# Dzh-16/FLASH-Viterbi

Hardware: AMD Instinct MI355X
Metric: trellis_cells_per_sec (higher is better)
Workload: dtype f32 scores (+f64 add per cell, rounded to f32 as the reference does)

## Files before the change

flash_viterbi_amd/build.py:

```python
import os
import shutil
import subprocess

PKG = os.path.dirname(os.path.abspath(__file__))
ROOT = os.path.dirname(PKG)
INCLUDE = os.path.join(ROOT, "include")
CSRC = os.path.join(PKG, "csrc")

HOST_LIB = os.path.join(PKG, "libfvhost.so")
HIP_LIB = os.path.join(PKG, "libflashvit.so")

HIP_SOURCES = ["fv_context.hip", "fv_full.hip", "fv_beam.hip", "fv_comm.hip", "fv_schedule.cpp"]
HIP_DEPS = ["fv_internal.h", "fv_layout.h", "fv_device_common.h", "fv_kernels.hip.inc", "fv_beam_kernels.hip.inc", "fv_schedule.h"]
OBJ_DIR = os.path.join(PKG, "_obj")
HIP_TIMING_LIB = os.path.join(PKG, "libflashvit_timing.so")


def _newer(target, sources):
    if not os.path.isfile(target):
        return False
    t = os.path.getmtime(target)
    return all(os.path.getmtime(s) <= t for s in sources if os.path.isfile(s))


def _run(cmd, cwd=None):
    res = subprocess.run(cmd, cwd=cwd, capture_output=True, text=True)
    if res.returncode != 0:
        raise RuntimeError("build failed: " + " ".join(cmd) + "\n" + res.stdout + res.stderr)
# ... 73 lines not shown
```

flash_viterbi_amd/csrc/fv_context.hip:

```cpp
#include "fv_internal.h"

namespace {

template <typename F>
void parallel_rows(int rows, F &&fn)
{
    unsigned hw = std::thread::hardware_concurrency();
    int nt = (int)std::min<unsigned>(hw ? hw : 4, 16);
    if (rows < 256) nt = 1;
    if (nt <= 1) { fn(0, rows); return; }
    std::vector<std::thread> th;
    int per = (rows + nt - 1) / nt;
    for (int t = 0; t < nt; ++t) {
        int a = t * per, b = std::min(rows, a + per);
        if (a >= b) break;
        th.emplace_back([=, &fn] { fn(a, b); });
    }
    for (auto &x : th) x.join();
}

}

namespace fvi {

size_t device_bytes(const fv_ctx *c)
{
    return c->LA32.bytes() + c->LA16.bytes() + c->LAQ16.bytes() + c->SPdata.bytes() + c->SPoff.bytes() + c->SPnwb.bytes() + c->LB32T.bytes() + c->LA64.bytes() + c->LB64T.bytes() + c->LPi64.bytes() +
           c->d_ob.bytes() + c->d_ans.bytes() + c->d_bp.bytes() + c->d_gather.bytes() + c->d_rows.bytes() + c->d_ckpt.bytes() +
           c->d_score.bytes() + c->d_counters.bytes() + c->d_hval.bytes() + c->d_scores.bytes() +
           c->d_hstate.bytes() + c->d_flags.bytes() + c->d_slot_val.bytes() + c->d_slot_state.bytes() +
           c->LA64R.bytes() + c->LAQ16R.bytes() + c->d_qaux.bytes() + c->d_tie_list.bytes() + c->d_tie_count.bytes() + c->d_cut.bytes() + c->d_dupwin.bytes() + c->d_cand.bytes() + c->d_cand_count.bytes() + c->d_passL.bytes() + c->d_needfull.bytes() + c->d_seqof.bytes() + c->d_doubt.bytes() + c->d_doubt_count.bytes() + c->d_pack.bytes() +
           c->CSk.bytes() + c->CSq.bytes() + c->CS64.bytes() + c->CSoff.bytes() + c->CSnwb.bytes() + c->CRptr.bytes() + c->CRcol.bytes() + c->CRlog.bytes();
}

inline size_t pack_head(int nscores) { return 2 * FV_NCOUNTERS + (size_t)std::max(4, round_up(nscores, 4)); }

size_t pack_ints(const fv_ctx *ctx, int T, int nscores) { return pack_head(nscores) + (size_t)T * std::max(1, ctx->nranks) + (size_t)T; }

int ensure_workspace(fv_ctx *ctx, int T, size_t rows_needed, int nscores)
{
    const size_t want_rows = rows_needed * 2 * (size_t)ctx->nrows;
    const size_t want_pack = pack_ints(ctx, T, nscores);
    if (nscores > 1) {
        unsigned long long grow = 0, released = 0;
// ... 231 lines not shown
        for (fv_ctx *m : g->members) m->group = nullptr;
        for (size_t r = g->members.size(); r-- > 1;) fv_destroy(g->members[r]);
        for (hipEvent_t e : g->ans_ready) if (e) (void)hipEventDestroy(e);
        delete g;
    }
    (void)hipSetDevice(ctx->device);
    if (ctx->stream) (void)hipStreamSynchronize(ctx->stream);
    if (ctx->comm) ncclCommDestroy(ctx->comm);
    ctx->LA32.release(); ctx->LA16.release(); ctx->LAQ16.release(); ctx->SPdata.release(); ctx->SPoff.release(); ctx->SPnwb.release(); ctx->LB32T.release(); ctx->LA64.release(); ctx->LB64T.release(); ctx->LPi64.release();
    ctx->d_ob.release(); ctx->d_ans.release(); ctx->d_bp.release(); ctx->d_gather.release(); ctx->d_rows.release(); ctx->d_ckpt.release();
    ctx->d_score.release(); ctx->d_counters.release(); ctx->d_hval.release(); ctx->d_scores.release();
    ctx->d_hstate.release(); ctx->d_flags.release(); ctx->d_slot_val.release(); ctx->d_slot_state.release();
    ctx->LA64R.release(); ctx->LAQ16R.release(); ctx->d_qaux.release(); ctx->d_tie_list.release(); ctx->d_tie_count.release(); ctx->d_cut.release(); ctx->d_dupwin.release(); ctx->d_cand.release(); ctx->d_cand_count.release(); ctx->d_passL.release(); ctx->d_needfull.release(); ctx->d_seqof.release(); ctx->d_doubt.release(); ctx->d_doubt_count.release(); ctx->d_pack.release();
    fvi::release_csr(ctx);
    if (ctx->h_pin) { (void)hipHostFree(ctx->h_pin); ctx->h_pin = nullptr; ctx->h_pin_n = 0; }
    for (hipEvent_t e : ctx->prof_events) (void)hipEventDestroy(e);
    if (ctx->ev_start) (void)hipEventDestroy(ctx->ev_start);
    if (ctx->ev_stop) (void)hipEventDestroy(ctx->ev_stop);
    if (ctx->ev_top) (void)hipEventDestroy(ctx->ev_top);
    if (ctx->ev_s0) (void)hipEventDestroy(ctx->ev_s0);
    if (ctx->ev_s1) (void)hipEventDestroy(ctx->ev_s1);
    if (ctx->ev_fork) (void)hipEventDestroy(ctx->ev_fork);
    for (int q = 0; q < fv_ctx::BEAM_AUX; ++q) {
        if (ctx->ev_join[q]) (void)hipEventDestroy(ctx->ev_join[q]);
        if (ctx->aux[q]) (void)hipStreamDestroy(ctx->aux[q]);
    }
    if (ctx->stream) (void)hipStreamDestroy(ctx->stream);
    delete ctx;
}

// ... 400 lines not shown
    if (ctx->group && ctx->group_rank == 0) {
        for (int r = fvi::group_size(ctx) - 1; r >= 1; --r) {
            const int rc = fv_set_option(fvi::group_member(ctx, r), key, value);
            if (rc) return rc;
        }
    }
    switch (key) {
    case FV_OPT_KERNEL:
        if (value < FV_KERNEL_AUTO || value > FV_KERNEL_U16_REFINE) return FV_ERR_ARG;
        ctx->opt_kernel = (int)value; return FV_OK;
    case FV_OPT_MAX_BATCH:
        if (value < 1 || value > fvk::MAX_BATCH) return FV_ERR_ARG;
        ctx->opt_max_batch = (int)value; return FV_OK;
    case FV_OPT_PROFILE:
        ctx->opt_profile = value ? 1 : 0; return FV_OK;
    case FV_OPT_SEL_MARGIN:
        if (value < 0 || value > 100000) return FV_ERR_ARG;
        ctx->opt_sel_margin = (float)value * 1e-3f; return FV_OK;
    case FV_OPT_DEBUG:
#ifndef FV_TIMING_BUILD
        if (value & FV_DEBUG_TIMING_ONLY) { ctx->detail = "FV_OPT_DEBUG: result-changing timing switches need the timing build"; return FV_ERR_ARG; }
#endif
        if (value < 0 || value >= (1ll << 32) || (value & ((1ll << 27) | (1ll << 30)))) return FV_ERR_ARG;
        ctx->opt_csr_mem = (int)((value >> 31) & 1);
        ctx->opt_debug = (int)(value & 0x3fffffff); return FV_OK;
    default: return FV_ERR_ARG;
    }
}

extern "C" long long fv_checkpoint_memory_bytes(int K, int T, int step)
// ... 50 lines not shown
```

flash_viterbi_amd/csrc/fv_full.hip:

```cpp
#include "fv_internal.h"
#include "fv_kernels.hip.inc"
#include "flashvit_testing.h"

namespace {

int pick_kernel(const fv_ctx *ctx)
{
    if (ctx->opt_kernel == FV_KERNEL_F64_STREAM) return FV_KERNEL_F64_STREAM;
    if (!ctx->logs_nonpositive) return FV_KERNEL_F64_STREAM;
    if (ctx->opt_kernel == FV_KERNEL_F16_REFINE || ctx->opt_kernel == FV_KERNEL_F32_REFINE ||
        ctx->opt_kernel == FV_KERNEL_Q16_REFINE || ctx->opt_kernel == FV_KERNEL_U16_REFINE)
        return ctx->opt_kernel;
    if (ctx->opt_kernel == FV_KERNEL_SPARSE_Q16) return ctx->SPdata.p ? FV_KERNEL_SPARSE_Q16 : FV_KERNEL_U16_REFINE;
    return (ctx->SPdata.p && ctx->density <= 0.35) ? FV_KERNEL_SPARSE_Q16 : FV_KERNEL_U16_REFINE;
}

constexpr int U_UP = 16, U_DB32 = 4, U_DB64 = 2, U_DB16 = 2;

constexpr int nb_slot(int NB) { return NB == 1 ? 0 : NB == 2 ? 1 : NB == 4 ? 2 : 3; }
template <typename TA> constexpr int tab_slot()
{
    return std::is_same<TA, double>::value ? 0 : std::is_same<TA, float>::value ? 1 : std::is_same<TA, fvk::half_t>::value ? 2 : 3;
}
template <typename TA, int NB, bool DB> constexpr unsigned long long step_variant()
// ... 255 lines not shown

struct ProfRange { size_t first, count; };

int prof_event(fv_ctx *ctx, size_t idx, hipEvent_t *out)
{
    while (ctx->prof_events.size() <= idx) {
        hipEvent_t e;
        FV_HIP(hipEventCreate(&e));
        ctx->prof_events.push_back(e);
    }
    *out = ctx->prof_events[idx];
    return 0;
}

enum { BATCH_NONE = 0, BATCH_SERIAL = 1, BATCH_FORK = 2 };
int run_generation_full(fv_ctx *ctx, std::vector<fv::Pass> &passes, int kernel, size_t &nprof, int batch = BATCH_NONE)
{
    const int K = ctx->K;
    const int np = (int)passes.size();
    if (np == 0) return 0;
    std::stable_sort(passes.begin(), passes.end(),
                     [](const fv::Pass &a, const fv::Pass &b) { return a.R - a.L > b.R - b.L; });
    for (int base = 0; base < np; base += fvk::PASS_CHUNK) {
        fvk::PassChunk ch;
        ch.n = std::min(fvk::PASS_CHUNK, np - base);
        for (int q = 0; q < ch.n; ++q) {
            const fv::Pass &p = passes[base + q];
            ch.p[q] = fvk::PassDesc{ p.L, p.R, p.from_pi ? 1 : 0, p.whole ? 1 : 0, (long long)(base + q) * 2 * ctx->nrows };
        }
        if (ctx->csr)
            hipLaunchKernelGGL(fvk::init_rows_csr, dim3((K + 255) / 256, ch.n), dim3(256), 0, ctx->stream, ch, ctx->CRptr.p,
                               ctx->CRcol.p, ctx->CRlog.p, ctx->LB64T.p, ctx->LPi64.p, ctx->d_ob.p, ctx->d_ans.p, ctx->d_rows.p, K);
        else
        hipLaunchKernelGGL(fvk::init_rows, dim3((K + 255) / 256, ch.n), dim3(256), 0, ctx->stream, ch,
                           ctx->LA64.p, ctx->nrows, ctx->LB64T.p, ctx->LPi64.p, ctx->d_ob.p, ctx->d_ans.p,
                           ctx->d_rows.p, K);
        FV_HIP(hipGetLastError());
    }
    const int maxlen = passes[0].R - passes[0].L;
    const bool slabbed = (kernel == FV_KERNEL_F64_STREAM || kernel == FV_KERNEL_Q16_REFINE) && !ctx->full_ok;
    int cap = std::max(1, std::min(ctx->opt_max_batch, slabbed ? 4 : max_batch_for(ctx->nrows, !ctx->full_ok)));
    if (kernel == FV_KERNEL_SPARSE_CSR) cap = ctx->opt_max_batch;
    const bool whole_gen = passes[0].whole;
    constexpr int FORK_STREAMS = 3, FORK_CAP = 4;
    const bool two = ((kernel == FV_KERNEL_U16_REFINE && ctx->u16_ok) || ((kernel == FV_KERNEL_SPARSE_Q16 || kernel == FV_KERNEL_SPARSE_CSR) && maxlen >= 64)) &&
                     !(ctx->opt_debug & 262144) && (!whole_gen || batch == BATCH_FORK) && np > FORK_CAP &&
                     !ctx->opt_profile && !(ctx->opt_debug & 64);
    const int nbatches = (np + FORK_CAP - 1) / FORK_CAP;
    const int nstreams = two ? std::min(FORK_STREAMS, nbatches) : 1;
    auto fork = [&]() -> int {
        FV_HIP(hipEventRecord(ctx->ev_fork, ctx->stream));
        for (int q = 1; q < nstreams; ++q) FV_HIP(hipStreamWaitEvent(ctx->aux[q - 1], ctx->ev_fork, 0));
        return 0;
// ... 5 lines not shown
            while ((qe = hipStreamQuery(ctx->stream)) == hipErrorNotReady) std::this_thread::yield();
            FV_HIP(qe);
        }
        ctx->fork_active = true;
        { int rc = fork(); if (rc) return rc; }
    }
    ctx->forked_batches = two;
    struct Unfork { fv_ctx *c; ~Unfork() { c->forked_batches = false; c->lstream = nullptr; } } unfork{ ctx };
    auto join = [&]() -> int {
        for (int q = 1; q < nstreams; ++q) {
            FV_HIP(hipEventRecord(ctx->ev_join[q - 1], ctx->aux[q - 1]));
            FV_HIP(hipStreamWaitEvent(ctx->stream, ctx->ev_join[q - 1], 0));
        }
        return 0;
    };
    const bool col_last = !(ctx->opt_debug & 8);
    const bool use_graph = (ctx->opt_debug & 64) && !ctx->opt_profile;
    if (use_graph) FV_HIP(hipStreamBeginCapture(ctx->stream, hipStreamCaptureModeThreadLocal));
    if (whole_gen && !use_graph) FV_HIP(hipEventRecord(ctx->ev_s0, ctx->stream));
    int active = np;
    for (int s = 1; s <= maxlen; ++s) {
        while (active > 0 && passes[active - 1].R - passes[active - 1].L < s) --active;
        int full = active;
        if (col_last) while (full > 0 && passes[full - 1].R - passes[full - 1].L == s && !passes[full - 1].whole) --full;
        auto row = [&](int q, int parity) { return ctx->d_rows.p + (size_t)q * 2 * ctx->nrows + (size_t)parity * ctx->nrows; };
        for (int base = 0; base < full; base += cap) {
            const int nb = std::min(cap, full - base);
            fvk::TaskSlot slots[fvk::MAX_BATCH];
            for (int q = 0; q < nb; ++q) {
                const fv::Pass &p = passes[base + q];
                slots[q].t1_in = row(base + q, (s - 1) & 1);
                slots[q].t1_out = row(base + q, s & 1);
                slots[q].tmp_row = ctx->LB32T.p + (size_t)ctx->h_ob[p.L + s] * K;
                slots[q].tmp64_row = ctx->LB64T.p + (size_t)ctx->h_ob[p.L + s] * K;
                slots[q].bp_out = ctx->d_bp.p + (size_t)(p.L + s) * K;
            }
// ... 41 lines not shown
            }
            int rc = flush();
            if (rc) return rc;
        }
    }
    if (use_graph) {
        hipGraph_t g = nullptr;
        FV_HIP(hipStreamEndCapture(ctx->stream, &g));
        hipGraphExec_t ge = nullptr;
        FV_HIP(hipGraphInstantiate(&ge, g, nullptr, nullptr, 0));
        if (whole_gen) FV_HIP(hipEventRecord(ctx->ev_s0, ctx->stream));
        FV_HIP(hipGraphLaunch(ge, ctx->stream));
        ctx->graphs.push_back(ge);
        (void)hipGraphDestroy(g);
    }
    if (whole_gen && !two) FV_HIP(hipEventRecord(ctx->ev_s1, ctx->stream));
    if (two) { int rc = join(); if (rc) return rc; }
    if (whole_gen && two) FV_HIP(hipEventRecord(ctx->ev_s1, ctx->stream));
    if (batch) {
        fvk::ArgmaxArgs a;
        a.rows = ctx->d_rows.p; a.ans = ctx->d_ans.p; a.score = ctx->d_score.p; a.K = K; a.nrows = ctx->nrows; a.n = 0;
        auto flush = [&]() -> int {
            if (a.n == 0) return 0;
            hipLaunchKernelGGL(fvk::final_argmax_batch, dim3(a.n), dim3(1024), 0, ctx->stream, a);
            FV_HIP(hipGetLastError());
            a.n = 0;
            return 0;
        };
        for (int q = 0; q < np; ++q) {
            if (!passes[q].whole) continue;
            const int len = passes[q].R - passes[q].L;
// ... 297 lines not shown
    for (int q = 0; q < np; ++q) {
        const fv::Pass &p = gen[(size_t)q];
        int c = 0;
        while (tp[c].L != p.L) ++c;
        const float *row = ctx->d_rows.p + (size_t)q * 2 * ctx->nrows + (size_t)((p.R - p.L) & 1) * ctx->nrows;
        FV_HIP(hipMemcpyAsync(rows_out + (size_t)c * K, row, (size_t)K * sizeof(float), hipMemcpyDeviceToHost, ctx->stream));
        FV_HIP(hipMemcpyAsync(bp_out + (size_t)(p.L + 1) * K, ctx->d_bp.p + (size_t)(p.L + 1) * K,
                              (size_t)(p.R - p.L) * K * sizeof(int), hipMemcpyDeviceToHost, ctx->stream));
    }
    FV_HIP(hipStreamSynchronize(ctx->stream));
    for (hipGraphExec_t ge : ctx->graphs) (void)hipGraphExecDestroy(ge);
    ctx->graphs.clear();
    if (variants_out) *variants_out = ctx->test_variants;
    return FV_OK;
}
}

extern "C" int fv_test_forward(fv_ctx *ctx, const int *ob, int T, const fv_test_pass *passes, int npasses,
                               float *rows_out, int *bp_out, unsigned long long *variants_out)
{
    if (!ctx) return FV_ERR_ARG;
    if (fvi::group_size(ctx) > 1) { ctx->detail = "fv_test_forward: one device per context"; return FV_ERR_ARG; }
    return fvi::drained(ctx, test_forward_impl(ctx, ob, T, passes, npasses, rows_out, bp_out, variants_out));
}

extern "C" int fv_decode_vanilla(fv_ctx *ctx, const int *ob, int T, int *path_out, float *score_out)
{
    if (!ctx) return FV_ERR_ARG;
    if (ctx->csr) { ctx->detail = "fv_decode_vanilla: not available on a model set by fv_set_model_sparse (its kernel reads the dense table)"; return FV_ERR_UNSUPPORTED; }
    const int keep_kernel = ctx->opt_kernel;
// ... 112 lines not shown
```

flash_viterbi_amd/csrc/fv_internal.h:

```cpp
#pragma once

#include <hip/hip_runtime.h>
#include <rccl/rccl.h>

#include <algorithm>
#include <chrono>
#include <condition_variable>
#include <functional>
#include <mutex>
#include <cmath>
#include <cstdio>
#include <cstdlib>
#include <cstring>
#include <string>
#include <thread>
#include <vector>

#include "flashvit.h"
#include "fv_layout.h"
#include "fv_schedule.h"

using clk = std::chrono::steady_clock;
inline double ms_since(clk::time_point t0) { return std::chrono::duration<double, std::milli>(clk::now() - t0).count(); }

// ... 42 lines not shown
    bool laq16_ready = false;
    DevBuf<double> LA64, LB64T, LPi64;
    bool csr = false;
    DevBuf<uint4> CSk;
    DevBuf<uint2> CSq;
    DevBuf<double> CS64;
    DevBuf<long long> CSoff;
    DevBuf<int> CSnwb;
    DevBuf<long long> CRptr;
    DevBuf<int> CRcol;
    DevBuf<double> CRlog;

    DevBuf<int> d_ob, d_ans, d_bp, d_gather;
    DevBuf<float> d_rows, d_score, d_ckpt;
    DevBuf<unsigned long long> d_counters;
    DevBuf<int> d_pack;
    int *h_pin = nullptr;
    size_t h_pin_n = 0;
    DevBuf<float> d_hval, d_scores, d_slot_val;
    DevBuf<int> d_hstate, d_slot_state, d_flags;
    DevBuf<double> LA64R;
    DevBuf<unsigned short> LAQ16R;
    bool rowq_ready = false, beam_q16_ready = false;
    DevBuf<unsigned long long> d_qaux;
    DevBuf<int2> d_tie_list;
    DevBuf<float> d_cut;
    DevBuf<fvb::HNode> d_cand;
    DevBuf<int> d_cand_count;
    float opt_sel_margin = 0.3f;
    DevBuf<int> d_dupwin;
    DevBuf<int> d_doubt, d_doubt_count;
    DevBuf<int> d_needfull;
    DevBuf<int> d_seqof;
    std::vector<int> h_seqof;
    DevBuf<int> d_passL;
    std::vector<int> h_passL;
    DevBuf<unsigned int> d_tie_count;

    int opt_kernel = FV_KERNEL_AUTO;
    int opt_max_batch = fvk::MAX_BATCH;
    int opt_profile = 0;
    int vanilla = 0;
    int opt_csr_mem = 0;
    int opt_debug = 0;
    std::vector<hipEvent_t> prof_events;
    std::vector<int> h_ob;
    std::vector<hipGraphExec_t> graphs;
    bool test_record = false;
    unsigned long long test_variants = 0;

    ncclComm_t comm = nullptr;
    int rank = 0, nranks = 1;
    struct fv_group *group = nullptr;
    int group_rank = 0;

    fv_stats stats{};
// ... 76 lines not shown
```

flash_viterbi_amd/decoder.py:

```python
import ctypes
import os

import numpy as np

from . import build as _build

MODE_REFERENCE = 0
MODE_SINGLE_PASS = 1
KERNEL_AUTO, KERNEL_F64_STREAM, KERNEL_F32_REFINE, KERNEL_F16_REFINE, KERNEL_Q16_REFINE, KERNEL_SPARSE_Q16 = 0, 1, 2, 3, 4, 5
KERNEL_U16_REFINE = 6
KERNEL_SPARSE_CSR = 7
OPT_KERNEL, OPT_MAX_BATCH, OPT_PROFILE, OPT_SEL_MARGIN, OPT_DEBUG = 1, 2, 3, 4, 100
DEBUG_TIMING_ONLY = (1 << 0) | (1 << 4) | (1 << 5) | (1 << 11) | (1 << 12)
DEBUG_BATCH_GEN0_SERIAL = 1 << 28
DEBUG_BEAM_BATCH_GEN0_OTHER = 1 << 29
DEBUG_CSR_ROWS_IN_MEMORY = 1 << 31
WARN_BEAM_MISS = 1
ERR_ARG, ERR_NOMEM, ERR_NO_PRED, ERR_DEVICE, ERR_STATE, ERR_UNSUPPORTED = -1, -2, -3, -4, -5, -6
UNIQUE_ID_BYTES = 128


class Stats(ctypes.Structure):
    _fields_ = [("set_model_ms", ctypes.c_double), ("decode_ms", ctypes.c_double), ("gpu_ms", ctypes.c_double),
                ("top_pass_ms", ctypes.c_double), ("top_steps_ms", ctypes.c_double),
                ("step_kernel_ms", ctypes.c_double),
                ("step_launches", ctypes.c_longlong), ("task_steps", ctypes.c_longlong),
                ("column_steps", ctypes.c_longlong),
# ... 11 lines not shown

    def as_dict(self):
        return {k: getattr(self, k) for k, _ in self._fields_}


class PassInfo(ctypes.Structure):
    _fields_ = [("L", ctypes.c_int), ("R", ctypes.c_int), ("generation", ctypes.c_int), ("owner", ctypes.c_int)]


EXPORTS = ["fv_create", "fv_destroy", "fv_set_model", "fv_set_option", "fv_decode_full", "fv_decode_beam",
           "fv_decode_vanilla", "fv_decode_checkpoint", "fv_checkpoint_memory_bytes",
           "fv_last_stats", "fv_strerror", "fv_last_error_detail", "fv_reference_memory_bytes",
           "fv_comm_unique_id", "fv_comm_init", "fv_plan_passes", "fv_merge_paths", "fv_set_partition",
           "fv_create_multi", "fv_device_count", "fv_decode_full_batch", "fv_plan_passes_batch", "fv_decode_beam_batch",
           "fv_set_model_sparse"]
TEST_EXPORTS = ["fv_test_forward", "fv_test_beam_step"]
TIE_TAG = 1 << 30


class ForwardPass(ctypes.Structure):
    _fields_ = [("L", ctypes.c_int), ("R", ctypes.c_int), ("init_state", ctypes.c_int)]


class BeamSet(ctypes.Structure):
    _fields_ = [("val", ctypes.c_void_p), ("state", ctypes.c_void_p), ("n", ctypes.c_int)]

_lib = None


def load_library():
    global _lib
# ... 23 lines not shown
    L.fv_checkpoint_memory_bytes.argtypes = [ci, ci, ci]
    L.fv_checkpoint_memory_bytes.restype = ctypes.c_longlong
    L.fv_last_stats.argtypes = [vp, ctypes.POINTER(Stats)]
    L.fv_strerror.argtypes = [ci]
    L.fv_strerror.restype = ctypes.c_char_p
    L.fv_last_error_detail.argtypes = [vp]
    L.fv_last_error_detail.restype = ctypes.c_char_p
    L.fv_reference_memory_bytes.argtypes = [ci, ci, ci, ci]
    L.fv_reference_memory_bytes.restype = cll
    L.fv_comm_unique_id.argtypes = [vp]
    L.fv_comm_init.argtypes = [vp, ci, ci, vp]
    L.fv_set_partition.argtypes = [vp, ci, ci]
    L.fv_plan_passes.argtypes = [ci, ci, ci, ci, ctypes.POINTER(PassInfo), ci]
    L.fv_merge_paths.argtypes = [ci, ci, ci, vp, vp]
    L.fv_test_forward.argtypes = [vp, vp, ci, ctypes.POINTER(ForwardPass), ci, vp, vp, ctypes.POINTER(ctypes.c_ulonglong)]
    cf = ctypes.c_float
    L.fv_test_beam_step.argtypes = [vp, ci, ctypes.POINTER(BeamSet), ci, vp, ci, cf, cf, ci, vp, vp, vp, ctypes.POINTER(ci),
                                    vp, vp, vp, vp, ctypes.POINTER(ctypes.c_ulonglong)]
    _lib = L
    return L


class FlashVitError(RuntimeError):
    def __init__(self, rc, detail=""):
        msg = load_library().fv_strerror(rc).decode()
        super().__init__(f"flashvit: {msg} ({rc})" + (f": {detail}" if detail else ""))
        self.rc = rc


def plan_passes(T, n_split, mode=MODE_REFERENCE, nranks=1):
# ... 150 lines not shown
    def decode_checkpoint(self, ob, step=0):
        ob = np.ascontiguousarray(ob, dtype=np.int32)
        path = np.empty(ob.size, dtype=np.int32)
        score = ctypes.c_float(0)
        rc = self._check(self._L.fv_decode_checkpoint(self._h, _p(ob), ob.size, step, _p(path), ctypes.byref(score)))
        return path, np.float32(score.value), rc

    def test_forward(self, ob, passes, bp_fill=-2):
        ob = np.ascontiguousarray(ob, dtype=np.int32)
        pa = (ForwardPass * len(passes))(*[ForwardPass(int(L), int(R), int(s)) for L, R, s in passes])
        rows = np.empty((len(passes), self.K), dtype=np.float32)
        bp = np.full((ob.size, self.K), bp_fill, dtype=np.int32)
        variants = ctypes.c_ulonglong(0)
        self._check(self._L.fv_test_forward(self._h, _p(ob), ob.size, pa, len(passes), _p(rows), _p(bp), ctypes.byref(variants)))
        return rows, bp, int(variants.value)

    def test_beam_step(self, beam, sets, syms, speculative=False, theta=0.0, next_bound=float("inf"), cand_cap=0):
        K = self.K
        vals = [np.ascontiguousarray(v, dtype=np.float32) for v, _ in sets]
        sts = [np.ascontiguousarray(s, dtype=np.int32) for _, s in sets]
        arr = (BeamSet * len(sets))(*[BeamSet(_p(v).value, _p(s).value, v.size) for v, s in zip(vals, sts)])
        syms = np.ascontiguousarray(syms, dtype=np.int32)
        n = len(sets)
        scores = np.empty((n, K), dtype=np.float32)
        bp = np.empty((n, K), dtype=np.int32)
        ties = np.empty((n * K, 2), dtype=np.int32)
        nties = ctypes.c_int(0)
        doubt = np.empty((n, 1024), dtype=np.int32)
        doubt_counts = np.empty(n, dtype=np.int32)
        cand = np.empty((n, max(cand_cap, 1), 2), dtype=np.int32)
# ... 38 lines not shown
```

include/flashvit.h:

```cpp
#ifndef FLASHVIT_H
#define FLASHVIT_H

#include <stddef.h>

#ifdef __cplusplus
extern "C" {
#endif

typedef struct fv_ctx fv_ctx;

enum {
    FV_OK = 0,
    FV_WARN_BEAM_MISS = 1,
    FV_ERR_ARG = -1,
    FV_ERR_NOMEM = -2,
    FV_ERR_NO_PRED = -3,
    FV_ERR_DEVICE = -4,
    FV_ERR_STATE = -5,
    FV_ERR_UNSUPPORTED = -6,
    FV_ERR_COMM = -7,
};

enum {
    FV_MODE_REFERENCE = 0,
    FV_MODE_SINGLE_PASS = 1,
};

enum {
    FV_OPT_KERNEL = 1,
    FV_OPT_MAX_BATCH = 2,
    FV_OPT_PROFILE = 3,
    FV_OPT_SEL_MARGIN = 4,
    FV_OPT_DEBUG = 100,
};
#define FV_DEBUG_TIMING_ONLY ((1 << 0) | (1 << 4) | (1 << 5) | (1 << 11) | (1 << 12))
enum {
    FV_KERNEL_AUTO = 0,
    FV_KERNEL_F64_STREAM = 1,
    FV_KERNEL_F32_REFINE = 2,
    FV_KERNEL_F16_REFINE = 3,
    FV_KERNEL_Q16_REFINE = 4,
    FV_KERNEL_U16_REFINE = 6,
    FV_KERNEL_SPARSE_Q16 = 5,
    FV_KERNEL_SPARSE_CSR = 7,
};

typedef struct {
// ... 88 lines not shown
```

include/flashvit_testing.h:

```cpp
#ifndef FLASHVIT_TESTING_H
#define FLASHVIT_TESTING_H

#include "flashvit.h"

#ifdef __cplusplus
extern "C" {
#endif

typedef struct { int L, R, init_state; } fv_test_pass;

int fv_test_forward(fv_ctx *ctx, const int *ob, int T, const fv_test_pass *passes, int npasses,
                    float *rows_out, int *bp_out, unsigned long long *variants_out);

typedef struct { const float *val; const int *state; int n; } fv_test_beam_set;
typedef struct { float value; int state; } fv_test_cand;

#define FV_TEST_TIE_TAG (1 << 30)
int fv_test_beam_step(fv_ctx *ctx, int beam, const fv_test_beam_set *sets, int nsets, const int *sym, int speculative,
                      float theta, float next_bound, int cand_cap, float *scores_out, int *bp_out, int *ties_out,
                      int *tie_count_out, int *doubt_out, int *doubt_counts, fv_test_cand *cand_out, int *cand_counts,
                      unsigned long long *variants_out);

#define FV_TV_F64_NB1        (1ull << 0)
#define FV_TV_F64_NB2        (1ull << 1)
#define FV_TV_F64_NB4        (1ull << 2)
#define FV_TV_F64_NB8        (1ull << 3)
#define FV_TV_F32_NB1        (1ull << 4)
// ... 60 lines not shown
```

Measured before the change: 1019 billion.

## Run whole-sequence top pass as one resident kernel with inter-block handover

Adds a persistent kernel that processes every time step of the single whole-sequence forward pass in one launch. Tiles exchange each step's row through a global handover buffer tagged with the step number instead of relying on one kernel launch per step. If a wait exceeds a wall-clock bound, a pinned host flag records the give-up and the pass is re-run per step, and the context stays on the per-step form from then on. The aim is to remove per-step launch and synchronisation overhead, at the risk of spin-wait stalls when there are more tiles than CUs, plus the added complexity of the fallback path.

New measurement: 1125 billion (median of 6 runs). 1.1x the previous value.

```diff
diff --git a/flash_viterbi_amd/build.py b/flash_viterbi_amd/build.py
--- a/flash_viterbi_amd/build.py
+++ b/flash_viterbi_amd/build.py
@@ -11,7 +11,7 @@
 HIP_LIB = os.path.join(PKG, "libflashvit.so")
 
 HIP_SOURCES = ["fv_context.hip", "fv_full.hip", "fv_beam.hip", "fv_comm.hip", "fv_schedule.cpp"]
-HIP_DEPS = ["fv_internal.h", "fv_layout.h", "fv_device_common.h", "fv_kernels.hip.inc", "fv_beam_kernels.hip.inc", "fv_schedule.h"]
+HIP_DEPS = ["fv_internal.h", "fv_layout.h", "fv_device_common.h", "fv_kernels.hip.inc", "fv_resident.hip.inc", "fv_beam_kernels.hip.inc", "fv_schedule.h"]
 OBJ_DIR = os.path.join(PKG, "_obj")
 HIP_TIMING_LIB = os.path.join(PKG, "libflashvit_timing.so")
 
diff --git a/flash_viterbi_amd/csrc/fv_context.hip b/flash_viterbi_amd/csrc/fv_context.hip
--- a/flash_viterbi_amd/csrc/fv_context.hip
+++ b/flash_viterbi_amd/csrc/fv_context.hip
@@ -27,7 +27,7 @@
 {
     return c->LA32.bytes() + c->LA16.bytes() + c->LAQ16.bytes() + c->SPdata.bytes() + c->SPoff.bytes() + c->SPnwb.bytes() + c->LB32T.bytes() + c->LA64.bytes() + c->LB64T.bytes() + c->LPi64.bytes() +
            c->d_ob.bytes() + c->d_ans.bytes() + c->d_bp.bytes() + c->d_gather.bytes() + c->d_rows.bytes() + c->d_ckpt.bytes() +
-           c->d_score.bytes() + c->d_counters.bytes() + c->d_hval.bytes() + c->d_scores.bytes() +
+           c->d_score.bytes() + c->d_counters.bytes() + c->d_handover.bytes() + c->d_hval.bytes() + c->d_scores.bytes() +
            c->d_hstate.bytes() + c->d_flags.bytes() + c->d_slot_val.bytes() + c->d_slot_state.bytes() +
            c->LA64R.bytes() + c->LAQ16R.bytes() + c->d_qaux.bytes() + c->d_tie_list.bytes() + c->d_tie_count.bytes() + c->d_cut.bytes() + c->d_dupwin.bytes() + c->d_cand.bytes() + c->d_cand_count.bytes() + c->d_passL.bytes() + c->d_needfull.bytes() + c->d_seqof.bytes() + c->d_doubt.bytes() + c->d_doubt_count.bytes() + c->d_pack.bytes() +
            c->CSk.bytes() + c->CSq.bytes() + c->CS64.bytes() + c->CSoff.bytes() + c->CSnwb.bytes() + c->CRptr.bytes() + c->CRcol.bytes() + c->CRlog.bytes();
@@ -289,6 +289,8 @@
     ctx->LA64R.release(); ctx->LAQ16R.release(); ctx->d_qaux.release(); ctx->d_tie_list.release(); ctx->d_tie_count.release(); ctx->d_cut.release(); ctx->d_dupwin.release(); ctx->d_cand.release(); ctx->d_cand_count.release(); ctx->d_passL.release(); ctx->d_needfull.release(); ctx->d_seqof.release(); ctx->d_doubt.release(); ctx->d_doubt_count.release(); ctx->d_pack.release();
     fvi::release_csr(ctx);
     if (ctx->h_pin) { (void)hipHostFree(ctx->h_pin); ctx->h_pin = nullptr; ctx->h_pin_n = 0; }
+    ctx->d_handover.release();
+    if (ctx->h_giveup) { (void)hipHostFree(ctx->h_giveup); ctx->h_giveup = nullptr; }
     for (hipEvent_t e : ctx->prof_events) (void)hipEventDestroy(e);
     if (ctx->ev_start) (void)hipEventDestroy(ctx->ev_start);
     if (ctx->ev_stop) (void)hipEventDestroy(ctx->ev_stop);
@@ -719,6 +721,9 @@
         ctx->opt_max_batch = (int)value; return FV_OK;
     case FV_OPT_PROFILE:
         ctx->opt_profile = value ? 1 : 0; return FV_OK;
+    case FV_OPT_TOP_PASS:
+        if (value < 0 || value > 3) return FV_ERR_ARG;
+        ctx->opt_top_pass = (int)value; return FV_OK;
     case FV_OPT_SEL_MARGIN:
         if (value < 0 || value > 100000) return FV_ERR_ARG;
         ctx->opt_sel_margin = (float)value * 1e-3f; return FV_OK;
diff --git a/flash_viterbi_amd/csrc/fv_full.hip b/flash_viterbi_amd/csrc/fv_full.hip
--- a/flash_viterbi_amd/csrc/fv_full.hip
+++ b/flash_viterbi_amd/csrc/fv_full.hip
@@ -1,5 +1,6 @@
 #include "fv_internal.h"
 #include "fv_kernels.hip.inc"
+#include "fv_resident.hip.inc"
 #include "flashvit_testing.h"
 
 namespace {
@@ -293,6 +294,58 @@
 }
 
 enum { BATCH_NONE = 0, BATCH_SERIAL = 1, BATCH_FORK = 2 };
+
+constexpr int RESIDENT_MIN_STEPS = 16;
+constexpr double RESIDENT_WAIT_MS = 4.0;
+
+bool resident_eligible(const fv_ctx *ctx, const std::vector<fv::Pass> &passes, int kernel, int batch)
+{
+    if (ctx->opt_top_pass == 1 || ctx->resident_off) return false;
+    if (batch != BATCH_NONE || passes.size() != 1 || !passes[0].whole) return false;
+    if (kernel != FV_KERNEL_U16_REFINE || !ctx->full_ok || ctx->vanilla || ctx->csr) return false;
+    const int ntiles = (ctx->K + fvk::TILE_W - 1) / fvk::TILE_W;
+    if (ntiles > ctx->num_cus || ctx->nrows > 4096 || (ctx->opt_debug & (4 | 8192))) return false;
+    if (ctx->opt_profile || (ctx->opt_debug & 64)) return false;
+    if (ctx->group && !ctx->group->rccl) return false;
+    return passes[0].R - passes[0].L >= RESIDENT_MIN_STEPS;
+}
+
+int run_top_pass_resident(fv_ctx *ctx, const fv::Pass &p, bool &gave_up)
+{
+    const int nrows = ctx->nrows, nsteps = p.R - p.L;
+    const size_t words = (size_t)2 * nrows + 2;
+    FV_HIP(ctx->d_handover.ensure(words));
+    if (!ctx->h_giveup) {
+        FV_HIP(hipHostMalloc(reinterpret_cast<void **>(&ctx->h_giveup), 64, hipHostMallocDefault));
+        FV_HIP(hipHostGetDevicePointer(reinterpret_cast<void **>(&ctx->d_giveup_view), ctx->h_giveup, 0));
+        int khz = 0;
+        if (hipDeviceGetAttribute(&khz, hipDeviceAttributeWallClockRate, ctx->device) != hipSuccess || khz <= 0) khz = 100000;
+        ctx->wall_clock_khz = khz;
+    }
+    *reinterpret_cast<volatile unsigned int *>(ctx->h_giveup) = 0u;
+    fvk::ResidentArgs a;
+    a.LA = ctx->LAQ16.p; a.LA64 = ctx->LA64.p; a.counters = ctx->d_counters.p; a.LB32T = ctx->LB32T.p; a.ob = ctx->d_ob.p;
+    a.bp = ctx->d_bp.p;
+    a.row_in = ctx->d_rows.p; a.row_last = ctx->d_rows.p + (size_t)(nsteps & 1) * nrows;
+    a.gran = ctx->d_handover.p; a.giveup_dev = reinterpret_cast<unsigned int *>(ctx->d_handover.p + (size_t)2 * nrows);
+    a.giveup_host = ctx->d_giveup_view;
+    a.spin_ticks = (long long)(RESIDENT_WAIT_MS * ctx->wall_clock_khz);
+    a.K = ctx->K; a.debug = ctx->opt_debug; a.nrows = nrows;
+    a.ntiles = (ctx->K + fvk::TILE_W - 1) / fvk::TILE_W; a.tiles_per_xcd = (a.ntiles + 7) / 8;
+    a.L = p.L; a.nsteps = nsteps;
+    a.window = ctx->windowq; a.qscale = ctx->qscale;
+    FV_HIP(hipMemsetAsync(ctx->d_handover.p, 0, words * sizeof(unsigned long long), ctx->stream));
+    FV_HIP(hipEventRecord(ctx->ev_s0, ctx->stream));
+    hipLaunchKernelGGL(fvk::trellis_pass_u16, dim3(a.tiles_per_xcd * 8), dim3(fvk::RES_THREADS), fvk::resident_lds_bytes(nrows), ctx->stream, a);
+    FV_HIP(hipGetLastError());
+    FV_HIP(hipEventRecord(ctx->ev_s1, ctx->stream));
+    hipError_t qe;
+    while ((qe = hipStreamQuery(ctx->stream)) == hipErrorNotReady) std::this_thread::yield();
+    FV_HIP(qe);
+    gave_up = *reinterpret_cast<volatile unsigned int *>(ctx->h_giveup) != 0u || ctx->opt_top_pass == 3;
+    return 0;
+}
+
 int run_generation_full(fv_ctx *ctx, std::vector<fv::Pass> &passes, int kernel, size_t &nprof, int batch = BATCH_NONE)
 {
     const int K = ctx->K;
@@ -300,22 +353,26 @@
     if (np == 0) return 0;
     std::stable_sort(passes.begin(), passes.end(),
                      [](const fv::Pass &a, const fv::Pass &b) { return a.R - a.L > b.R - b.L; });
-    for (int base = 0; base < np; base += fvk::PASS_CHUNK) {
-        fvk::PassChunk ch;
-        ch.n = std::min(fvk::PASS_CHUNK, np - base);
-        for (int q = 0; q < ch.n; ++q) {
-            const fv::Pass &p = passes[base + q];
-            ch.p[q] = fvk::PassDesc{ p.L, p.R, p.from_pi ? 1 : 0, p.whole ? 1 : 0, (long long)(base + q) * 2 * ctx->nrows };
-        }
-        if (ctx->csr)
-            hipLaunchKernelGGL(fvk::init_rows_csr, dim3((K + 255) / 256, ch.n), dim3(256), 0, ctx->stream, ch, ctx->CRptr.p,
-                               ctx->CRcol.p, ctx->CRlog.p, ctx->LB64T.p, ctx->LPi64.p, ctx->d_ob.p, ctx->d_ans.p, ctx->d_rows.p, K);
-        else
-        hipLaunchKernelGGL(fvk::init_rows, dim3((K + 255) / 256, ch.n), dim3(256), 0, ctx->stream, ch,
-                           ctx->LA64.p, ctx->nrows, ctx->LB64T.p, ctx->LPi64.p, ctx->d_ob.p, ctx->d_ans.p,
-                           ctx->d_rows.p, K);
-        FV_HIP(hipGetLastError());
-    }
+    auto init_all = [&]() -> int {
+        for (int base = 0; base < np; base += fvk::PASS_CHUNK) {
+            fvk::PassChunk ch;
+            ch.n = std::min(fvk::PASS_CHUNK, np - base);
+            for (int q = 0; q < ch.n; ++q) {
+                const fv::Pass &p = passes[base + q];
+                ch.p[q] = fvk::PassDesc{ p.L, p.R, p.from_pi ? 1 : 0, p.whole ? 1 : 0, (long long)(base + q) * 2 * ctx->nrows };
+            }
+            if (ctx->csr)
+                hipLaunchKernelGGL(fvk::init_rows_csr, dim3((K + 255) / 256, ch.n), dim3(256), 0, ctx->stream, ch, ctx->CRptr.p,
+                                   ctx->CRcol.p, ctx->CRlog.p, ctx->LB64T.p, ctx->LPi64.p, ctx->d_ob.p, ctx->d_ans.p, ctx->d_rows.p, K);
+            else
+            hipLaunchKernelGGL(fvk::init_rows, dim3((K + 255) / 256, ch.n), dim3(256), 0, ctx->stream, ch,
+                               ctx->LA64.p, ctx->nrows, ctx->LB64T.p, ctx->LPi64.p, ctx->d_ob.p, ctx->d_ans.p,
+                               ctx->d_rows.p, K);
+            FV_HIP(hipGetLastError());
+        }
+        return 0;
+    };
+    { int rc = init_all(); if (rc) return rc; }
     const int maxlen = passes[0].R - passes[0].L;
     const bool slabbed = (kernel == FV_KERNEL_F64_STREAM || kernel == FV_KERNEL_Q16_REFINE) && !ctx->full_ok;
     int cap = std::max(1, std::min(ctx->opt_max_batch, slabbed ? 4 : max_batch_for(ctx->nrows, !ctx->full_ok)));
@@ -351,12 +408,33 @@
         }
         return 0;
     };
+    bool resident_done = false;
+    if (whole_gen) ctx->top_pass_form = FV_TOP_PASS_PER_STEP;
+    if (resident_eligible(ctx, passes, kernel, batch)) {
+        bool gave_up = false;
+        int rc = run_top_pass_resident(ctx, passes[0], gave_up);
+        if (rc) return rc;
+        if (gave_up) {
+            if (ctx->opt_top_pass != 3) {
+                ctx->resident_off = true;
+                ctx->detail = "the resident launch of the whole-sequence pass gave up (a wait exceeded its bound): the pass was re-run with one launch per step, and this context keeps that form from now on";
+            }
+            ctx->top_pass_form = FV_TOP_PASS_RESIDENT_RERUN;
+            FV_HIP(hipMemsetAsync(ctx->d_counters.p, 0, FV_NCOUNTERS * sizeof(unsigned long long), ctx->stream));
+            if ((rc = init_all())) return rc;
+        } else {
+            resident_done = true;
+            ctx->top_pass_form = FV_TOP_PASS_RESIDENT;
+            ctx->stats.step_launches += maxlen;
+            ctx->stats.task_steps += maxlen;
+        }
+    }
     const bool col_last = !(ctx->opt_debug & 8);
     const bool use_graph = (ctx->opt_debug & 64) && !ctx->opt_profile;
     if (use_graph) FV_HIP(hipStreamBeginCapture(ctx->stream, hipStreamCaptureModeThreadLocal));
-    if (whole_gen && !use_graph) FV_HIP(hipEventRecord(ctx->ev_s0, ctx->stream));
+    if (whole_gen && !use_graph && !resident_done) FV_HIP(hipEventRecord(ctx->ev_s0, ctx->stream));
     int active = np;
-    for (int s = 1; s <= maxlen; ++s) {
+    for (int s = 1; s <= maxlen && !resident_done; ++s) {
         while (active > 0 && passes[active - 1].R - passes[active - 1].L < s) --active;
         int full = active;
         if (col_last) while (full > 0 && passes[full - 1].R - passes[full - 1].L == s && !passes[full - 1].whole) --full;
@@ -428,7 +506,7 @@
         ctx->graphs.push_back(ge);
         (void)hipGraphDestroy(g);
     }
-    if (whole_gen && !two) FV_HIP(hipEventRecord(ctx->ev_s1, ctx->stream));
+    if (whole_gen && !two && !resident_done) FV_HIP(hipEventRecord(ctx->ev_s1, ctx->stream));
     if (two) { int rc = join(); if (rc) return rc; }
     if (whole_gen && two) FV_HIP(hipEventRecord(ctx->ev_s1, ctx->stream));
     if (batch) {
@@ -756,6 +834,56 @@
     if (variants_out) *variants_out = ctx->test_variants;
     return FV_OK;
 }
+int test_top_pass_impl(fv_ctx *ctx, const int *ob, const long long *offsets, int nseq, int form, int *bp_out, float *rows_out,
+                       int *form_out)
+{
+    if (!ob || !offsets || nseq < 1 || form < 0 || form > 3 || !bp_out || !rows_out || offsets[0] != 0) return FV_ERR_ARG;
+    if (ctx->K == 0) return FV_ERR_STATE;
+    const int K = ctx->K;
+    std::vector<fv::Pass> gen((size_t)nseq);
+    for (int q = 0; q < nseq; ++q) {
+        const long long len = offsets[q + 1] - offsets[q];
+        if (len < 2 || offsets[q + 1] > 0x7fffffffLL) { ctx->detail = "fv_test_top_pass: every sequence needs 2 .. 2^31 - 1 observations"; return FV_ERR_ARG; }
+        gen[(size_t)q] = fv::Pass{ (int)offsets[q], (int)offsets[q + 1] - 1, true, true, 0, -1, q };
+    }
+    const int sumT = (int)offsets[nseq];
+    int kernel = FV_KERNEL_AUTO;
+    int rc = prepare_full(ctx, ob, sumT, (size_t)nseq, kernel, nseq > 1 ? nseq : 1);
+    if (rc) return rc;
+    reset_stats(ctx, kernel, 1);
+    ctx->stats.passes = nseq;
+    if ((rc = fvi::begin_decode(ctx, ob, sumT))) return rc;
+    struct Restore {
+        fv_ctx *c; int top;
+        ~Restore() { c->opt_top_pass = top; }
+    } restore{ ctx, ctx->opt_top_pass };
+    ctx->opt_top_pass = form;
+    ctx->fork_active = false;
+    size_t nprof = 0;
+    const int batch = nseq == 1 ? BATCH_NONE : (ctx->opt_debug & (1 << 28)) ? BATCH_SERIAL : BATCH_FORK;
+    if ((rc = run_generation_full(ctx, gen, kernel, nprof, batch))) return rc;
+    for (int q = 0; q < nseq; ++q) {
+        const fv::Pass &p = gen[(size_t)q];
+        const float *row = ctx->d_rows.p + (size_t)q * 2 * ctx->nrows + (size_t)((p.R - p.L) & 1) * ctx->nrows;
+        FV_HIP(hipMemcpyAsync(rows_out + (size_t)p.seq * K, row, (size_t)K * sizeof(float), hipMemcpyDeviceToHost, ctx->stream));
+        FV_HIP(hipMemcpyAsync(bp_out + (size_t)(p.L + 1) * K, ctx->d_bp.p + (size_t)(p.L + 1) * K,
+                              (size_t)(p.R - p.L) * K * sizeof(int), hipMemcpyDeviceToHost, ctx->stream));
+    }
+    FV_HIP(hipStreamSynchronize(ctx->stream));
+    for (hipStream_t a : ctx->aux) if (a) FV_HIP(hipStreamSynchronize(a));
+    for (hipGraphExec_t ge : ctx->graphs) (void)hipGraphExecDestroy(ge);
+    ctx->graphs.clear();
+    if (form_out) *form_out = ctx->top_pass_form;
+    return FV_OK;
+}
+}
+
+extern "C" int fv_test_top_pass(fv_ctx *ctx, const int *ob, const long long *offsets, int nseq, int form, int *bp_out,
+                                float *rows_out, int *form_out)
+{
+    if (!ctx) return FV_ERR_ARG;
+    if (fvi::group_size(ctx) > 1) { ctx->detail = "fv_test_top_pass: one device per context"; return FV_ERR_ARG; }
+    return fvi::drained(ctx, test_top_pass_impl(ctx, ob, offsets, nseq, form, bp_out, rows_out, form_out));
 }
 
 extern "C" int fv_test_forward(fv_ctx *ctx, const int *ob, int T, const fv_test_pass *passes, int npasses,
diff --git a/flash_viterbi_amd/csrc/fv_internal.h b/flash_viterbi_amd/csrc/fv_internal.h
--- a/flash_viterbi_amd/csrc/fv_internal.h
+++ b/flash_viterbi_amd/csrc/fv_internal.h
@@ -80,6 +80,11 @@
     DevBuf<int> d_ob, d_ans, d_bp, d_gather;
     DevBuf<float> d_rows, d_score, d_ckpt;
     DevBuf<unsigned long long> d_counters;
+    DevBuf<unsigned long long> d_handover;
+    unsigned int *h_giveup = nullptr, *d_giveup_view = nullptr;
+    int wall_clock_khz = 100000;
+    bool resident_off = false;
+    int top_pass_form = 0;
     DevBuf<int> d_pack;
     int *h_pin = nullptr;
     size_t h_pin_n = 0;
@@ -106,6 +111,7 @@
     int opt_kernel = FV_KERNEL_AUTO;
     int opt_max_batch = fvk::MAX_BATCH;
     int opt_profile = 0;
+    int opt_top_pass = 0;
     int vanilla = 0;
     int opt_csr_mem = 0;
     int opt_debug = 0;
diff --git a/flash_viterbi_amd/csrc/fv_resident.hip.inc b/flash_viterbi_amd/csrc/fv_resident.hip.inc
--- /dev/null
+++ b/flash_viterbi_amd/csrc/fv_resident.hip.inc
@@ -0,0 +1,310 @@
+#pragma once
+
+namespace fvk {
+
+struct ResidentArgs {
+    const void *LA;
+    const double *LA64;
+    unsigned long long *counters;
+    const float *LB32T;
+    const int *ob;
+    int *bp;
+    const float *row_in;
+    float *row_last;
+    unsigned long long *gran;
+    unsigned int *giveup_dev;
+    unsigned int *giveup_host;
+    long long spin_ticks;
+    int K, debug, nrows, ntiles, tiles_per_xcd;
+    int L, nsteps;
+    float window, qscale;
+};
+
+constexpr int RES_NWV = 8, RES_U = 16, RES_THREADS = RES_NWV * 64;
+
+static inline size_t resident_lds_bytes(int nrows)
+{
+    return (size_t)nrows * 2 + (size_t)nrows * 4 + (size_t)RES_NWV * TILE_W * 12 + 16;
+}
+
+__global__ __launch_bounds__(RES_THREADS) void trellis_pass_u16(const ResidentArgs args)
+{
+    constexpr int R = 8, RBR = 32, NWV = RES_NWV, U = RES_U;
+    typedef __attribute__((address_space(1))) unsigned long long gu64;
+    typedef __attribute__((address_space(1))) unsigned int gu32;
+    extern __shared__ __align__(16) unsigned char smem[];
+    const int nrows = args.nrows, npairs = nrows >> 1;
+    unsigned int *T1c = reinterpret_cast<unsigned int *>(smem);
+    float *T1f = reinterpret_cast<float *>(T1c + npairs);
+    unsigned int *redZ = reinterpret_cast<unsigned int *>(T1f + nrows);
+    float *redR = reinterpret_cast<float *>(redZ + NWV * TILE_W);
+    int *redK = reinterpret_cast<int *>(redR + NWV * TILE_W);
+    unsigned int *wg_fail = reinterpret_cast<unsigned int *>(redK + NWV * TILE_W);
+
+    const int tid = threadIdx.x, lane = tid & 63, w = tid >> 6;
+    const int c = lane & (TILE_W - 1), rg = lane >> 4;
+    const int tile = (blockIdx.x & 7) * args.tiles_per_xcd + (blockIdx.x >> 3);
+    if (tile >= args.ntiles) return;
+    const int col = tile * TILE_W + c;
+    const int K = args.K;
+    const unsigned short *tile_base = reinterpret_cast<const unsigned short *>(args.LA) + (size_t)tile * nrows * TILE_W;
+    const uint4 *LAt = reinterpret_cast<const uint4 *>(tile_base) + rg * TILE_W + c;
+    const int nq = nrows / RBR;
+    const int nj = nq > w ? (nq - w + NWV - 1) / NWV : 0;
+    const float step = -args.qscale, inv_step = 1.0f / step;
+    const double *L64tile = args.LA64 + (size_t)tile * nrows * TILE_W;
+    const double *L64t = L64tile + c * 4;
+    const int blk0 = nj > 0 ? w : 0;
+
+    uint4 cur[U];
+#pragma unroll
+    for (int u = 0; u < U; ++u)
+        cur[u] = u < nj ? LAt[(size_t)(w + NWV * u) * (4 * TILE_W)] : make_uint4(0xffffffffu, 0xffffffffu, 0xffffffffu, 0xffffffffu);
+    if (tid == 0) *wg_fail = 0u;
+    __syncthreads();
+
+    gu64 *const gran = (gu64 *)args.gran;
+    gu32 *const giveup_dev = (gu32 *)args.giveup_dev;
+
+    for (int s = 1; s <= args.nsteps; ++s) {
+        const float tmp = args.LB32T[(size_t)args.ob[args.L + s] * K + min(col, K - 1)];
+        float v[8];
+        if (s == 1) {
+#pragma unroll
+            for (int h = 0; h < 4; ++h) {
+                const int p = h * RES_THREADS + tid;
+                const float2 x = p < npairs ? reinterpret_cast<const float2 *>(args.row_in)[p] : make_float2(0.f, 0.f);
+                v[2 * h] = x.x; v[2 * h + 1] = x.y;
+            }
+        } else {
+            const gu64 *g = gran + (size_t)((s - 1) & 1) * nrows;
+            const unsigned int want = (unsigned int)(s - 1);
+            long long t0 = 0;
+            for (unsigned int spins = 0;; ++spins) {
+                unsigned long long x[8];
+#pragma unroll
+                for (int e = 0; e < 8; ++e) {
+                    const int k = 2 * ((e >> 1) * RES_THREADS + tid) + (e & 1);
+                    x[e] = __hip_atomic_load(g + min(k, K - 1), __ATOMIC_RELAXED, __HIP_MEMORY_SCOPE_AGENT);
+                }
+                bool ok = true;
+#pragma unroll
+                for (int e = 0; e < 8; ++e) {
+                    const int k = 2 * ((e >> 1) * RES_THREADS + tid) + (e & 1);
+                    v[e] = k < K ? __uint_as_float((unsigned int)x[e]) : 0.0f;
+                    ok &= k >= K || (unsigned int)(x[e] >> 32) == want;
+                }
+                if (__all(ok)) break;
+                const long long now = (long long)wall_clock64();
+                if (spins == 0) t0 = now;
+                bool leave = now - t0 > args.spin_ticks;
+                if (leave) {
+                    if (lane == 0) {
+                        __hip_atomic_store(giveup_dev, 1u, __ATOMIC_RELAXED, __HIP_MEMORY_SCOPE_AGENT);
+                        __hip_atomic_store(args.giveup_host, 1u, __ATOMIC_RELAXED, __HIP_MEMORY_SCOPE_SYSTEM);
+                    }
+                } else if ((spins & 31u) == 31u) {
+                    leave = __hip_atomic_load(giveup_dev, __ATOMIC_RELAXED, __HIP_MEMORY_SCOPE_AGENT) != 0u;
+                }
+                if (leave) {
+                    if (lane == 0) __hip_atomic_store(wg_fail, 1u, __ATOMIC_RELAXED, __HIP_MEMORY_SCOPE_WORKGROUP);
+                    break;
+                }
+                __builtin_amdgcn_s_sleep(1);
+            }
+        }
+        float Mx;
+        {
+            float *redM = reinterpret_cast<float *>(redZ);
+            float pm = FV_NEG_INF;
+#pragma unroll
+            for (int e = 0; e < 8; ++e) {
+                const int k = 2 * ((e >> 1) * RES_THREADS + tid) + (e & 1);
+                pm = k < K ? fmaxf(pm, v[e]) : pm;
+            }
+#pragma unroll
+            for (int m = 1; m < 64; m <<= 1) pm = fmaxf(pm, __shfl_xor(pm, m));
+            if (lane == 0) redM[w] = pm;
+            __syncthreads();
+            if (__hip_atomic_load(wg_fail, __ATOMIC_RELAXED, __HIP_MEMORY_SCOPE_WORKGROUP) != 0u) return;
+            float x = redM[lane & (NWV - 1)];
+#pragma unroll
+            for (int m = 1; m < NWV; m <<= 1) x = fmaxf(x, __shfl_xor(x, m));
+            Mx = x;
+#pragma unroll
+            for (int h = 0; h < 4; ++h) {
+                const int p = h * RES_THREADS + tid;
+                if (p < npairs) {
+                    T1c[p] = score_code(Mx, v[2 * h], inv_step) | (score_code(Mx, v[2 * h + 1], inv_step) << 16);
+                    *reinterpret_cast<float2 *>(T1f + 2 * p) = make_float2(v[2 * h], v[2 * h + 1]);
+                }
+            }
+        }
+        __syncthreads();
+
+        unsigned int m1p = 0xffffffffu, m2p = 0xffffffffu;
+        int alo = -1, ahi = -1;
+        if (!FV_TIMING_BIT(args.debug, 2048)) {
+#pragma unroll
+            for (int u = 0; u < U; ++u) {
+                if (u < nj) {
+                    const int qb = w + NWV * u;
+                    const unsigned int ca[4] = { cur[u].x, cur[u].y, cur[u].z, cur[u].w };
+                    const int pb = qb * (RBR / 2) + rg * (R / 2);
+                    const uint4 ct4 = *reinterpret_cast<const uint4 *>(T1c + pb);
+                    const unsigned int ct[4] = { ct4.x, ct4.y, ct4.z, ct4.w };
+                    const unsigned int old = m1p;
+#pragma unroll
+                    for (int i = 0; i < 4; ++i) {
+                        const unsigned int z = pk_adds(ca[i], ct[i]);
+                        m2p = pk_minu(m2p, pk_maxu(z, m1p));
+                        m1p = pk_minu(m1p, z);
+                    }
+                    const unsigned int x = m1p ^ old;
+                    alo = (x & 0xffffu) ? qb : alo;
+                    ahi = (x >> 16) ? qb : ahi;
+                }
+            }
+        }
+        const unsigned int lo = m1p & 0xffffu, hi = m1p >> 16;
+        const int par = hi < lo ? 1 : 0;
+        const unsigned int m1 = par ? hi : lo;
+        int a1 = par ? ahi : alo;
+        const unsigned int m2 = min(max(lo, hi), min(m2p & 0xffffu, m2p >> 16));
+        {
+            const int blk = a1 >= 0 ? a1 : blk0;
+            const int pos = (blk - w) / NWV;
+            uint4 ce = cur[0];
+#pragma unroll
+            for (int u = 1; u < U; ++u) {
+                const bool hit = u == pos;
+                ce.x = hit ? cur[u].x : ce.x; ce.y = hit ? cur[u].y : ce.y; ce.z = hit ? cur[u].z : ce.z; ce.w = hit ? cur[u].w : ce.w;
+            }
+            const unsigned int ca[4] = { ce.x, ce.y, ce.z, ce.w };
+            const uint4 ct4 = *reinterpret_cast<const uint4 *>(T1c + blk * (RBR / 2) + rg * (R / 2));
+            const unsigned int ct[4] = { ct4.x, ct4.y, ct4.z, ct4.w };
+            const int k0 = blk * RBR + rg * R;
+            int found = k0 + par;
+#pragma unroll
+            for (int i = 3; i >= 0; --i) {
+                const unsigned int z = pk_adds(ca[i], ct[i]);
+                const unsigned int zh = par ? (z >> 16) : (z & 0xffffu);
+                found = zh == m1 ? k0 + 2 * i + par : found;
+            }
+            a1 = a1 >= 0 ? found : -1;
+        }
+
+        unsigned int Zc;
+        {
+            unsigned int x = m1;
+            x = min(x, (unsigned int)__shfl_xor((int)x, 16));
+            x = min(x, (unsigned int)__shfl_xor((int)x, 32));
+            if (lane < TILE_W) redZ[c * NWV + w] = x;
+        }
+        __syncthreads();
+        {
+            const uint4 *q = reinterpret_cast<const uint4 *>(redZ + c * NWV);
+            unsigned int x = 0xffffffffu;
+#pragma unroll
+            for (int y = 0; y < NWV / 4; ++y) {
+                const uint4 f = q[y];
+                x = min(min(x, min(f.x, f.y)), min(f.z, f.w));
+            }
+            Zc = x;
+        }
+
+        float rr = FV_NEG_INF;
+        int rk = INT_MAX;
+        {
+            int kind = 0;
+            if (col < K && !FV_TIMING_BIT(args.debug, 4096)) {
+                const float zz = fabsf(Mx + tmp) + 65536.0f * step + 1.0f;
+                const unsigned int eb = __float_as_uint(zz) & 0x7f800000u;
+                const float Uf = (eb > (24u << 23) && eb < 0x7f800000u) ? __uint_as_float(eb - (23u << 23)) : (eb >= 0x7f800000u ? 0.0f : FLT_MIN);
+                const float wf = (2.0f * Uf + args.window) * inv_step + 3.1f;
+                const unsigned int W = wf < 65535.0f ? (unsigned int)wf + 1u : 65535u;
+                const unsigned int thr = Zc + W;
+                if (thr >= 65535u) {
+                    kind = 2;
+                    if (w == 0 && rg == 0) atomicAdd(&args.counters[8], 1ull);
+                }
+                else if (m2 <= thr) kind = 2;
+                else if (m1 <= thr && a1 >= 0) kind = 1;
+            }
+            if (kind == 1) {
+                const double Lc = L64t[(size_t)(a1 >> 2) * (TILE_W * 4) + (a1 & 3)];
+                const float tv = T1f[a1];
+                rr = exact_cell(tmp, tv, Lc);
+                rk = a1;
+                if (m1 != Zc) atomicAdd(&args.counters[0], 1ull);
+            }
+            unsigned long long need = __ballot(kind == 2);
+            while (need) {
+                const int Ln = __ffsll((long long)need) - 1;
+                need &= need - 1;
+                const int cL = Ln & (TILE_W - 1), rgL = Ln >> 4;
+                const float tmpL = __shfl(tmp, Ln);
+                float bx = FV_NEG_INF;
+                int bk = INT_MAX;
+                const int nlane_rows = nj * R;
+                for (int e0 = 0; e0 < nlane_rows; e0 += 128) {
+                    int kk[2];
+                    float tt[2];
+                    double LL[2];
+#pragma unroll
+                    for (int u = 0; u < 2; ++u) {
+                        const int e = e0 + 64 * u + lane;
+                        const int k = (w + NWV * (e / R)) * RBR + rgL * R + (e % R);
+                        kk[u] = (e < nlane_rows && k < K) ? k : -1;
+                        const int ks = kk[u] >= 0 ? k : 0;
+                        tt[u] = T1f[ks];
+                        LL[u] = L64tile[(size_t)(ks >> 2) * (TILE_W * 4) + cL * 4 + (ks & 3)];
+                    }
+#pragma unroll
+                    for (int u = 0; u < 2; ++u) {
+                        if (kk[u] >= 0) {
+                            const float x = exact_cell(tmpL, tt[u], LL[u]);
+                            if (better(x, kk[u], bx, bk)) { bx = x; bk = kk[u]; }
+                        }
+                    }
+                }
+#pragma unroll
+                for (int m = 1; m < 64; m <<= 1) {
+                    const float ov = __shfl_xor(bx, m);
+                    const int ok = __shfl_xor(bk, m);
+                    if (better(ov, ok, bx, bk)) { bx = ov; bk = ok; }
+                }
+                if (lane == Ln) { rr = bx; rk = bk; }
+                if (lane == 0) atomicAdd(&args.counters[1], 1ull);
+            }
+        }
+
+        {
+            float r = rr;
+            int kb = rk;
+            wave_best(r, kb);
+            if (lane < TILE_W) { redR[c * NWV + w] = r; redK[c * NWV + w] = kb; }
+        }
+        __syncthreads();
+        if (w == 0) {
+            const float4 fv = *reinterpret_cast<const float4 *>(redR + c * NWV + (rg * 4) % NWV);
+            const int4 fk = *reinterpret_cast<const int4 *>(redK + c * NWV + (rg * 4) % NWV);
+            float r = fv.x;
+            int kb = fk.x;
+            if (better(fv.y, fk.y, r, kb)) { r = fv.y; kb = fk.y; }
+            if (better(fv.z, fk.z, r, kb)) { r = fv.z; kb = fk.z; }
+            if (better(fv.w, fk.w, r, kb)) { r = fv.w; kb = fk.w; }
+            wave_best(r, kb);
+            const bool any = r > -FLT_MAX;
+            if (lane < TILE_W && col < K) {
+                const float out = any ? r : -FLT_MAX;
+                __hip_atomic_store(gran + (size_t)(s & 1) * nrows + col, ((unsigned long long)(unsigned int)s << 32) | __float_as_uint(out),
+                                   __ATOMIC_RELAXED, __HIP_MEMORY_SCOPE_AGENT);
+                args.bp[(size_t)(args.L + s) * K + col] = any ? kb : -1;
+                if (s == args.nsteps) args.row_last[col] = out;
+            }
+        }
+    }
+}
+
+}
diff --git a/flash_viterbi_amd/decoder.py b/flash_viterbi_amd/decoder.py
--- a/flash_viterbi_amd/decoder.py
+++ b/flash_viterbi_amd/decoder.py
@@ -11,6 +11,8 @@
 KERNEL_U16_REFINE = 6
 KERNEL_SPARSE_CSR = 7
 OPT_KERNEL, OPT_MAX_BATCH, OPT_PROFILE, OPT_SEL_MARGIN, OPT_DEBUG = 1, 2, 3, 4, 100
+OPT_TOP_PASS = 5
+TOP_PASS_PER_STEP, TOP_PASS_RESIDENT, TOP_PASS_RESIDENT_RERUN = 1, 2, 3
 DEBUG_TIMING_ONLY = (1 << 0) | (1 << 4) | (1 << 5) | (1 << 11) | (1 << 12)
 DEBUG_BATCH_GEN0_SERIAL = 1 << 28
 DEBUG_BEAM_BATCH_GEN0_OTHER = 1 << 29
@@ -52,7 +54,7 @@
            "fv_comm_unique_id", "fv_comm_init", "fv_plan_passes", "fv_merge_paths", "fv_set_partition",
            "fv_create_multi", "fv_device_count", "fv_decode_full_batch", "fv_plan_passes_batch", "fv_decode_beam_batch",
            "fv_set_model_sparse"]
-TEST_EXPORTS = ["fv_test_forward", "fv_test_beam_step"]
+TEST_EXPORTS = ["fv_test_forward", "fv_test_beam_step", "fv_test_top_pass"]
 TIE_TAG = 1 << 30
 
 
@@ -106,6 +108,7 @@
     L.fv_plan_passes.argtypes = [ci, ci, ci, ci, ctypes.POINTER(PassInfo), ci]
     L.fv_merge_paths.argtypes = [ci, ci, ci, vp, vp]
     L.fv_test_forward.argtypes = [vp, vp, ci, ctypes.POINTER(ForwardPass), ci, vp, vp, ctypes.POINTER(ctypes.c_ulonglong)]
+    L.fv_test_top_pass.argtypes = [vp, vp, vp, ci, ci, vp, vp, ctypes.POINTER(ci)]
     cf = ctypes.c_float
     L.fv_test_beam_step.argtypes = [vp, ci, ctypes.POINTER(BeamSet), ci, vp, ci, cf, cf, ci, vp, vp, vp, ctypes.POINTER(ci),
                                     vp, vp, vp, vp, ctypes.POINTER(ctypes.c_ulonglong)]
@@ -286,6 +289,18 @@
         variants = ctypes.c_ulonglong(0)
         self._check(self._L.fv_test_forward(self._h, _p(ob), ob.size, pa, len(passes), _p(rows), _p(bp), ctypes.byref(variants)))
         return rows, bp, int(variants.value)
+
+    def test_top_pass(self, obs, form, bp_fill=-2):
+        single = not isinstance(obs, (list, tuple))
+        seqs = [np.ascontiguousarray(o, dtype=np.int32).reshape(-1) for o in ([obs] if single else obs)]
+        offsets = np.zeros(len(seqs) + 1, dtype=np.int64)
+        offsets[1:] = np.cumsum([o.size for o in seqs])
+        ob = np.concatenate(seqs)
+        bp = np.full((ob.size, self.K), bp_fill, dtype=np.int32)
+        rows = np.empty((len(seqs), self.K), dtype=np.float32)
+        ran = ctypes.c_int(0)
+        self._check(self._L.fv_test_top_pass(self._h, _p(ob), _p(offsets), len(seqs), int(form), _p(bp), _p(rows), ctypes.byref(ran)))
+        return bp, rows, int(ran.value)
 
     def test_beam_step(self, beam, sets, syms, speculative=False, theta=0.0, next_bound=float("inf"), cand_cap=0):
         K = self.K
diff --git a/include/flashvit.h b/include/flashvit.h
--- a/include/flashvit.h
+++ b/include/flashvit.h
@@ -31,6 +31,7 @@
     FV_OPT_MAX_BATCH = 2,
     FV_OPT_PROFILE = 3,
     FV_OPT_SEL_MARGIN = 4,
+    FV_OPT_TOP_PASS = 5,
     FV_OPT_DEBUG = 100,
 };
 #define FV_DEBUG_TIMING_ONLY ((1 << 0) | (1 << 4) | (1 << 5) | (1 << 11) | (1 << 12))
diff --git a/include/flashvit_testing.h b/include/flashvit_testing.h
--- a/include/flashvit_testing.h
+++ b/include/flashvit_testing.h
@@ -11,6 +11,13 @@
 
 int fv_test_forward(fv_ctx *ctx, const int *ob, int T, const fv_test_pass *passes, int npasses,
                     float *rows_out, int *bp_out, unsigned long long *variants_out);
+
+#define FV_TOP_PASS_PER_STEP       1
+#define FV_TOP_PASS_RESIDENT       2
+#define FV_TOP_PASS_RESIDENT_RERUN 3
+
+int fv_test_top_pass(fv_ctx *ctx, const int *ob, const long long *offsets, int nseq, int form, int *bp_out,
+                     float *rows_out, int *form_out);
 
 typedef struct { const float *val; const int *state; int n; } fv_test_beam_set;
 typedef struct { float value; int state; } fv_test_cand;
```
